# imazen/image-webp

Hardware: AMD Instinct MI355X
Metric: 1920x1080 lossy encodes/s (Q75, method 4) (higher is better)
Workload: dtype int32; 1 GPU; encode_frame_lossy 1920x1080 RGBA Q75 m4; device_batch=1024, distinct_frames=4, mbs_per_frame=8160, parallelism=frames sharded over 1 GPU(s), steps_pipelined=True, pipeline_lanes=2

## Files before the change

image-webp_amd/csrc/zw_enc_kernels.hip:

```cpp
#include "zw_dev.h"

#include "zw_enc_rows.h"

#ifdef ZW_NW
#define ZW_NW1 ZW_NW
#define ZW_NW2 ZW_NW
#endif
#ifndef ZW_NW1
#define ZW_NW1 12
#endif
#ifndef ZW_NW2
#define ZW_NW2 12
#endif
#define NW_MAX (ZW_NW1 > ZW_NW2 ? ZW_NW1 : ZW_NW2)
#ifndef ZW_DYN_PRIO
#define ZW_DYN_PRIO 1
#endif
#ifndef ZW_DYN_PRIO1
#define ZW_DYN_PRIO1 2
#endif
#ifndef ZW_P1_LUMA_MAX
#define ZW_P1_LUMA_MAX 3
#endif
#ifndef ZW_CHAIN_PRIO
#define ZW_CHAIN_PRIO 3
#endif
#ifndef ZW_LUMA_PRIO
#define ZW_LUMA_PRIO 0
#endif
#ifndef ZW_UVQ_CHAIN_ROWS
#define ZW_UVQ_CHAIN_ROWS 1
#endif
#ifndef ZW_UVQ_CHAIN_BATCH
#define ZW_UVQ_CHAIN_BATCH 0
#endif
#ifndef ZW_PAIR_UNROLL
#define ZW_PAIR_UNROLL 1
#endif
#ifndef ZW_FETCH_AHEAD
#define ZW_FETCH_AHEAD (PASS == 2)
#endif
#ifndef ZW_AN4_GPW
#define ZW_AN4_GPW 1
#endif

template <int PASS> struct PassShape {
    static constexpr int NW = PASS == 1 ? ZW_NW1 : ZW_NW2;
    static constexpr int WG = NW * 64;
};

__device__ __forceinline__ int rgb_y(const uint8_t* p)
{
    return (16839 * p[0] + 33059 * p[1] + 6420 * p[2] + (1 << 15) + (16 << 16)) >> 16;
}
__device__ __forceinline__ int rgb_u(const uint8_t* p) { return -9719 * p[0] - 19081 * p[1] + 28800 * p[2] + (128 << 16); }
__device__ __forceinline__ int rgb_v(const uint8_t* p) { return 28800 * p[0] - 24116 * p[1] - 4684 * p[2] + (128 << 16); }

__device__ __forceinline__ void rgb2yuv_sample(const uint8_t* __restrict__ im, int w, int h, int bpp, int mbw, int cx,
                                               int cy, uint8_t* __restrict__ Yf, uint8_t* __restrict__ Uf,
                                               uint8_t* __restrict__ Vf)
{
    const int cw = mbw * 8, lw = mbw * 16;
    const int acw = (w + 1) / 2, ach = (h + 1) / 2;
    const int scx = cx < acw ? cx : acw - 1, scy = cy < ach ? cy : ach - 1;
    int xs[2] = {min(2 * scx, w - 1), min(2 * scx + 1, w - 1)};
    int ys[2] = {min(2 * scy, h - 1), min(2 * scy + 1, h - 1)};
#pragma unroll
    for (int dy = 0; dy < 2; dy++)
#pragma unroll
        for (int dx = 0; dx < 2; dx++) {
            int px = min(2 * cx + dx, w - 1), py = min(2 * cy + dy, h - 1);
            const uint8_t* p = im + ((size_t)py * w + px) * bpp;
            Yf[(size_t)(2 * cy + dy) * lw + 2 * cx + dx] = (uint8_t)(bpp <= 2 ? p[0] : rgb_y(p));
        }
    uint8_t uo = 127, vo = 127;
    if (bpp > 2) {
        int su = 0, sv = 0;
#pragma unroll
        for (int dy = 0; dy < 2; dy++)
#pragma unroll
            for (int dx = 0; dx < 2; dx++) {
                const uint8_t* p = im + ((size_t)ys[dy] * w + xs[dx]) * bpp;
                su += rgb_u(p);
                sv += rgb_v(p);
            }
        uo = (uint8_t)((su + (1 << 17)) >> 18);
        vo = (uint8_t)((sv + (1 << 17)) >> 18);
    }
    Uf[(size_t)cy * cw + cx] = uo;
    Vf[(size_t)cy * cw + cx] = vo;
}

extern "C" __global__ void k_rgb2yuv(const uint8_t* __restrict__ img, int w, int h, int bpp, int mbw, int mbh,
                                     uint8_t* __restrict__ Y, uint8_t* __restrict__ U, uint8_t* __restrict__ V,
                                     size_t img_stride, size_t ysz, size_t csz)
{
    const int cw = mbw * 8, chh = mbh * 8;
    const int f = blockIdx.y;
    const int idx = blockIdx.x * blockDim.x + threadIdx.x;
    if (idx >= cw * chh) return;
    rgb2yuv_sample(img + (size_t)f * img_stride, w, h, bpp, mbw, idx % cw, idx / cw, Y + (size_t)f * ysz,
                   U + (size_t)f * csz, V + (size_t)f * csz);
}

template <int BPP>
__device__ __forceinline__ void rgb_run8(const uint8_t* __restrict__ row, uint32_t px[8])
{
    typedef uint32_t u32x4 __attribute__((ext_vector_type(4)));
    typedef uint32_t u32x2 __attribute__((ext_vector_type(2)));
    if (BPP == 4) {
        const u32x4 a = __builtin_nontemporal_load((const u32x4*)row);
        const u32x4 b = __builtin_nontemporal_load((const u32x4*)(row + 16));
        px[0] = a.x; px[1] = a.y; px[2] = a.z; px[3] = a.w;
        px[4] = b.x; px[5] = b.y; px[6] = b.z; px[7] = b.w;
    } else {
        const u32x2 a = __builtin_nontemporal_load((const u32x2*)row);
        const u32x2 b = __builtin_nontemporal_load((const u32x2*)(row + 8));
        const u32x2 c = __builtin_nontemporal_load((const u32x2*)(row + 16));
        const uint32_t wd[6] = {a.x, a.y, b.x, b.y, c.x, c.y};
#pragma unroll
        for (int q = 0; q < 2; q++) {
            const uint32_t w0 = wd[3 * q], w1 = wd[3 * q + 1], w2 = wd[3 * q + 2];
            px[4 * q] = w0;
            px[4 * q + 1] = __builtin_amdgcn_alignbyte(w1, w0, 3);
            px[4 * q + 2] = __builtin_amdgcn_alignbyte(w2, w1, 2);
            px[4 * q + 3] = w2 >> 8;
        }
    }
}

template <int BPP>
__global__ __launch_bounds__(256) void k_rgb2yuv_rows(const uint8_t* __restrict__ img, int w, int h, int mbw, int mbh,
                                                      uint8_t* __restrict__ Y, uint8_t* __restrict__ U,
                                                      uint8_t* __restrict__ V, size_t img_stride, size_t ysz,
                                                      size_t csz)
{
    const int cw = mbw * 8, chh = mbh * 8, lw = mbw * 16, gpr = mbw * 2;
    const int f = blockIdx.y;
    const int idx = blockIdx.x * blockDim.x + threadIdx.x;
    if (idx >= gpr * chh) return;
    const int g = idx % gpr, cy = idx / gpr;
    const int cx0 = 4 * g, px0 = 8 * g;
    const uint8_t* im = img + (size_t)f * img_stride;
    uint8_t* Yf = Y + (size_t)f * ysz;
    uint8_t* Uf = U + (size_t)f * csz;
    uint8_t* Vf = V + (size_t)f * csz;
    if (px0 + 8 <= w && cy < (h + 1) / 2) {
        const int r0 = 2 * cy, r1 = min(2 * cy + 1, h - 1);
        uint32_t a[8], b[8];
        rgb_run8<BPP>(im + ((size_t)r0 * w + px0) * BPP, a);
        rgb_run8<BPP>(im + ((size_t)r1 * w + px0) * BPP, b);
        const uint32_t ya[2] = {pk_y4(a[0], a[1], a[2], a[3]), pk_y4(a[4], a[5], a[6], a[7])};
        const uint32_t yb[2] = {pk_y4(b[0], b[1], b[2], b[3]), pk_y4(b[4], b[5], b[6], b[7])};
        uint32_t uw = 0, vw = 0;
#pragma unroll
        for (int j = 0; j < 4; j++) {
            const int su = pk_u(a[2 * j]) + pk_u(a[2 * j + 1]) + pk_u(b[2 * j]) + pk_u(b[2 * j + 1]) + (512 << 16);
            const int sv = pk_v(a[2 * j]) + pk_v(a[2 * j + 1]) + pk_v(b[2 * j]) + pk_v(b[2 * j + 1]) + (512 << 16);
            uw |= (uint32_t)((su + (1 << 17)) >> 18) << (8 * j);
            vw |= (uint32_t)((sv + (1 << 17)) >> 18) << (8 * j);
        }
        *(uint2*)(Yf + (size_t)(2 * cy) * lw + px0) = make_uint2(ya[0], ya[1]);
        *(uint2*)(Yf + (size_t)(2 * cy + 1) * lw + px0) = make_uint2(yb[0], yb[1]);
        *(uint32_t*)(Uf + (size_t)cy * cw + cx0) = uw;
        *(uint32_t*)(Vf + (size_t)cy * cw + cx0) = vw;
    } else {
#pragma unroll
        for (int j = 0; j < 4; j++) rgb2yuv_sample(im, w, h, BPP, mbw, cx0 + j, cy, Yf, Uf, Vf);
    }
}

struct AnalysisTile {
    uint32_t y[16][4];
    uint32_t c[2][8][2];
    uint32_t ytop[4], ctop[2][2];
    uint8_t yleft[16], cleft[2][8];
    uint8_t corner[4];
};

DI void an_item(const AnalysisTile* A, bool luma, int mode, int b, bool ht, bool hl, int bins[16], int& z, int& vmax)
{
    const int pl = b >> 2;
    const int bb = luma ? b : (b & 3);
    const int bx = luma ? (bb & 3) : (bb & 1), by = luma ? (bb >> 2) : (bb >> 1);
    uint32_t st = 0, sl = 0;
    if (luma) {
#pragma unroll
        for (int w = 0; w < 4; w++) {
            st = __builtin_amdgcn_sad_u8(A->ytop[w], 0u, st);
            sl = __builtin_amdgcn_sad_u8(((const uint32_t*)A->yleft)[w], 0u, sl);
        }
    } else {
#pragma unroll
        for (int w = 0; w < 2; w++) {
            st = __builtin_amdgcn_sad_u8(A->ctop[pl][w], 0u, st);
            sl = __builtin_amdgcn_sad_u8(((const uint32_t*)A->cleft[pl])[w], 0u, sl);
        }
    }
    const uint32_t s2 = ht && hl ? st + sl : (ht ? 2 * st : 2 * sl);
    const int dcv = (ht || hl) ? (luma ? (int)((s2 + 16) >> 5) : (int)((s2 + 8) >> 4)) : 0x80;
    const int corner = A->corner[luma ? 0 : 1 + pl];
    int d[16];
#pragma unroll
    for (int i = 0; i < 4; i++) {
        const int r = by * 4 + i;
        const uint32_t srow = luma ? A->y[r][bx] : A->c[pl][r][bx];
        const int L = luma ? A->yleft[r] : A->cleft[pl][r];
#pragma unroll
        for (int j = 0; j < 4; j++) {
            const int cidx = bx * 4 + j;
            const uint32_t tw = luma ? A->ytop[cidx >> 2] : A->ctop[pl][cidx >> 2];
            const int T = (int)((tw >> (8 * (cidx & 3))) & 255u);
            const int tm = (ht && hl) ? clamp255(L + T - corner) : (hl ? L : (ht ? T : 129));
            const int p = mode == 0 ? dcv : tm;
            d[i * 4 + j] = (int)((srow >> (8 * j)) & 255u) - p;
        }
    }
    int o[16];
    fdct16_pk(d, o);
    z = 0;
    vmax = 0;
#pragma unroll
    for (int k = 0; k < 16; k++) {
        bins[k] = min(iabs(o[k]) >> 3, 31);
        z += bins[k] == 0;
        vmax = max(vmax, bins[k]);
    }
}
DI int max8(int v)
{
    v = max(v, DPP(v, 0xB1));
    v = max(v, DPP(v, 0x4E));
    return max(v, DPP(v, 0x141));
}
DI int an_red8(int v)
{
    v += DPP(v, 0xB1);
    v += DPP(v, 0x4E);
    return v + DPP(v, 0x141);
}
DI int max16(int v)
{
    v = max8(v);
    return max(v, DPP(v, 0x140));
}
typedef unsigned an_v4u __attribute__((ext_vector_type(4)));
typedef unsigned an_v2u __attribute__((ext_vector_type(2)));
extern "C" __global__ __launch_bounds__(256) void k_analysis4(const uint8_t* __restrict__ Y, const uint8_t* __restrict__ U,
                                                              const uint8_t* __restrict__ V, int mbw, int mbh,
                                                              size_t ysz, size_t csz, uint8_t* __restrict__ alpha,
                                                              uint32_t* __restrict__ histo)
{
    __shared__ AnalysisTile tile[4][4];
    __shared__ uint32_t hist[4][4][4][32];
    __shared__ uint32_t ahist[256];
    const int wv = threadIdx.x >> 6, lane = threadIdx.x & 63, mi = lane >> 4, j = lane & 15;
    const int f = blockIdx.y;
    const int nmb = mbw * mbh;
    ahist[threadIdx.x] = 0;
    __syncthreads();
    const int ys = mbw * 16, cs = mbw * 8;
    const uint8_t* Yf = Y + (size_t)f * ysz;
    const uint8_t* Uf = U + (size_t)f * csz;
    const uint8_t* Vf = V + (size_t)f * csz;
    AnalysisTile* A = &tile[wv][mi];
#pragma unroll 1
    for (int it = 0; it < ZW_AN4_GPW; it++) {
        const int mb = ((blockIdx.x * ZW_AN4_GPW + it) * 4 + wv) * 4 + mi;
        const bool in = mb < nmb;
        const int mbx = in ? mb % mbw : 0, mby = in ? mb / mbw : 0;
        const bool ht = mby > 0, hl = mbx > 0;
        {
            const int pl = j >> 3, cr = j & 7;
            const uint8_t* Cf = pl ? Vf : Uf;
            an_v4u yr = {0u, 0u, 0u, 0u};
            an_v2u cw = {0u, 0u};
            uint32_t yl = 0, cl = 0;
            if (in) {
                const uint8_t* yp = Yf + (size_t)(mby * 16 + j) * ys + mbx * 16;
                const uint8_t* cp = Cf + (size_t)(mby * 8 + cr) * cs + mbx * 8;
                yr = *(const an_v4u*)yp;
                cw = *(const an_v2u*)cp;
                if (hl) {
                    yl = yp[-1];
                    cl = cp[-1];
                }
            }
            wsync();
            *(an_v4u*)A->y[j] = yr;
            *(an_v2u*)A->c[pl][cr] = cw;
            A->yleft[j] = (uint8_t)yl;
            A->cleft[pl][cr] = (uint8_t)cl;
            if (j < 6) {
                uint32_t t0 = 0, t1 = 0, t2 = 0, t3 = 0;
                if (in && ht) {
                    if (j == 0) {
                        const an_v4u t = *(const an_v4u*)(Yf + (size_t)(mby * 16 - 1) * ys + mbx * 16);
                        t0 = t.x; t1 = t.y; t2 = t.z; t3 = t.w;
                    } else if (j < 3) {
                        const an_v2u t = *(const an_v2u*)((j == 1 ? Uf : Vf) + (size_t)(mby * 8 - 1) * cs + mbx * 8);
                        t0 = t.x; t1 = t.y;
                    } else if (hl) {
                        const uint8_t* cp = j == 3 ? Yf + (size_t)(mby * 16 - 1) * ys + mbx * 16 - 1
// ... 2092 lines not shown

struct MbFetch {
    uint32_t y, c;
    int alpha;
};
__device__ __forceinline__ MbFetch fetch_mb(const EncArgs* a, int f, int lane, int mbx, int mby)
{
    const int ys = a->mbw * 16, cs = a->mbw * 8;
    const uint8_t* sy = a->Y + (size_t)f * a->ysz + (size_t)mby * 16 * ys + mbx * 16;
    MbFetch r;
    r.y = *(const uint32_t*)(sy + (size_t)(lane >> 2) * ys + (lane & 3) * 4);
    r.c = 0;
    if (lane < 32) {
        const int pl = lane >> 4, k = lane & 15;
        const uint8_t* sp = (pl ? a->V : a->U) + (size_t)f * a->csz + (size_t)mby * 8 * cs + mbx * 8;
        r.c = *(const uint32_t*)(sp + (size_t)(k >> 1) * cs + (k & 1) * 4);
    }
    r.alpha = a->alpha[(size_t)f * a->mbw * a->mbh + (size_t)mby * a->mbw + mbx];
    return r;
}

__device__ void setup_ctx(Ctx& C, const EncArgs* a, const uint8_t* seg_lut, WaveLds* W, int mbx, int mby,
                          const MbFetch& m)
{
    C.mbx = mbx;
    C.mby = mby;
    const int f = C.f;
    C.ys = a->mbw * 16;
    C.cs = a->mbw * 8;
    C.srcY = a->Y + (size_t)f * a->ysz + (size_t)mby * 16 * C.ys + mbx * 16;
    C.srcU = a->U + (size_t)f * a->csz + (size_t)mby * 8 * C.cs + mbx * 8;
    C.srcV = a->V + (size_t)f * a->csz + (size_t)mby * 8 * C.cs + mbx * 8;
    {
        const int l = C.lane;
        ((uint32_t*)C.M->sy)[l] = m.y;
        if (l < 32) ((uint32_t*)((l >> 4) ? C.M->sv : C.M->su))[l & 15] = m.c;
        C.sY = C.M->sy;
        C.sU = C.M->su;
        C.sV = C.M->sv;
    }
    wsync();
    const int seg = __builtin_amdgcn_readfirstlane((int)seg_lut[m.alpha]);
    C.seg = seg;
    C.S = C.Sl + seg;
}

__device__ void wait_row(const int* progress, int wave_of_prev, int need)
{
    while (__hip_atomic_load(&progress[wave_of_prev], __ATOMIC_ACQUIRE, __HIP_MEMORY_SCOPE_WORKGROUP) < need)
        __builtin_amdgcn_s_sleep(1);
}
DI void set_prio(int p)
{
    if (p >= 3) __builtin_amdgcn_s_setprio(3);
    else if (p == 2) __builtin_amdgcn_s_setprio(2);
    else if (p == 1) __builtin_amdgcn_s_setprio(1);
    else __builtin_amdgcn_s_setprio(0);
}
__device__ void publish(int* progress, int wave, int val)
{
    __builtin_amdgcn_fence(__ATOMIC_RELEASE, "workgroup");
    if ((threadIdx.x & 63) == 0) __hip_atomic_store(&progress[wave], val, __ATOMIC_RELEASE, __HIP_MEMORY_SCOPE_WORKGROUP);
    __builtin_amdgcn_wave_barrier();
}


__device__ __forceinline__ int opaque_lane(int lane)
{
    asm volatile("" : "+v"(lane));
    return lane;
}

struct RowsLayout {
    size_t sync, ty, tu, tv, tc, td, frame;
    __host__ __device__ RowsLayout(int mbw, int mbh)
    {
        auto a16 = [](size_t v) { return (v + 15) & ~(size_t)15; };
        sync = 0;
        ty = a16(4 * (4 + (size_t)mbh));
        tu = ty + a16((size_t)mbw * 16 + 16);
        tv = tu + a16((size_t)mbw * 8);
        tc = tv + a16((size_t)mbw * 8);
        td = tc + a16((size_t)mbw * 12);
        frame = td + a16((size_t)mbw * 4);
    }
};
#define ZW_ROWS_HDR 256
#define ZW_ENC_SPIN_MAX (1 << 22)
DI uint32_t ld_sc1(const void* p) { return __hip_atomic_load((const uint32_t*)p, __ATOMIC_RELAXED, __HIP_MEMORY_SCOPE_AGENT); }
DI void st_sc1(void* p, uint32_t v) { __hip_atomic_store((uint32_t*)p, v, __ATOMIC_RELAXED, __HIP_MEMORY_SCOPE_AGENT); }
DI int row_ticket(int* ticket)
{
    int t = 0;
    if ((threadIdx.x & 63) == 0) t = atomicAdd(ticket, 1);
    return __builtin_amdgcn_readfirstlane(__shfl(t, 0));
}
DI void row_wait(const int* prog, int need, int* err, int& seen)
{
    if (seen >= need) return;
    int it = 0;
    for (;;) {
        seen = __builtin_amdgcn_readfirstlane((int)ld_sc1(prog));
        if (seen >= need) break;
        __builtin_amdgcn_s_sleep(1);
        if (++it > ZW_ENC_SPIN_MAX || ((it & 1023) == 0 && ld_sc1(err))) {
            if ((threadIdx.x & 63) == 0) atomicOr(err, 1);
            seen = 1 << 30;
            break;
        }
    }
    __builtin_amdgcn_fence(__ATOMIC_ACQUIRE, "agent");
}
DI void row_publish(int* prog, int val)
{
    asm volatile("s_waitcnt vmcnt(0)" ::: "memory");
    if ((threadIdx.x & 63) == 0)
        __hip_atomic_store((uint32_t*)prog, (uint32_t)val, __ATOMIC_RELEASE, __HIP_MEMORY_SCOPE_AGENT);
    __builtin_amdgcn_wave_barrier();
}

template <bool ROWS> struct ChainShape {
    static constexpr int NCH = (ROWS ? ZW_UVQ_CHAIN_ROWS : ZW_UVQ_CHAIN_BATCH) ? 2 : 1;
};
#if ZW_PAIR_UNROLL
#define ZW_PAIR_LOOP _Pragma("unroll")
#else
#define ZW_PAIR_LOOP _Pragma("nounroll")
#endif
template <int PASS> struct RowsShape {
    static constexpr int NW = PASS == 1 ? ChainShape<true>::NCH : 1;
};

constexpr size_t a16(size_t v) { return (v + 15) & ~(size_t)15; }

struct EncLds {
    static constexpr size_t sT = a16(sizeof(LdsTables)), sS = a16(4 * sizeof(ZwSegment)), sL = 256;
    static constexpr size_t sW = a16(sizeof(WaveLds)), sM = a16(sizeof(MbLds));
    size_t sy, su, sv, sc, sd;
    static constexpr size_t sProgress = 64, sXch = 256;
    __host__ __device__ EncLds(int mbw, bool rows, int pass)
    {
        const bool all = !rows, chain = rows && pass == 1;
        sy = all ? (((size_t)mbw * 16 + 48 + 15) & ~(size_t)15) : 0;
        su = sv = all || chain ? (((size_t)mbw * 8 + 48 + 15) & ~(size_t)15) : 0;
        sc = all ? (((size_t)mbw * 12 + 15) & ~(size_t)15) : 0;
        sd = all || chain ? (((size_t)mbw * 4 + 15) & ~(size_t)15) : 0;
    }
    __host__ __device__ size_t bytes(int nw, int fp) const
    {
        return sT * fp + sS * fp + sL * fp + sW * nw + (fp == 2 ? sM * nw : 0) + sProgress + sXch +
               (sy + su + sv + sc + sd) * fp;
    }
};
static_assert(NW_MAX * sizeof(int) <= 64, "the progress words");

DI void row_start(MbLds* M, int lane)
{
    if (lane < 20) M->left_y[lane] = 129;
    if (lane < 12) {
        M->left_u[lane] = 129;
        M->left_v[lane] = 129;
        M->left_c[lane] = 0;
    }
    if (lane < 4) M->left_derr[lane] = 0;
}

template <int PASS> DI void luma_issue_prio(const int* progress, int prevw, int mbx, int mby, int mbw)
{
#if ZW_DYN_PRIO > 0
    int slack = mbw;
    if (mby > 0) {
        const int v = __builtin_amdgcn_readfirstlane(
            __hip_atomic_load(&progress[prevw], __ATOMIC_RELAXED, __HIP_MEMORY_SCOPE_WORKGROUP));
        if ((v >> 16) == mby - 1) slack = (v & 0xffff) - mbx - 1;
    }
    constexpr int dp = PASS == 1 ? ZW_DYN_PRIO1 : ZW_DYN_PRIO;
    const int p = slack >= dp * 3 ? 3 : (slack >= dp * 2 ? 2 : (slack >= dp ? 1 : 0));
    set_prio(PASS == 1 ? min(p, ZW_P1_LUMA_MAX) : p);
#endif
}

template <int PASS, bool ROWS, int FP = 1>
__device__ __forceinline__ void encode_body(const EncArgs& a)
{
    constexpr int NW = ROWS ? RowsShape<PASS>::NW : PassShape<PASS>::NW, WG = NW * 64;
    constexpr int NCH = PASS == 1 ? ChainShape<ROWS>::NCH : 0;
    constexpr bool PAIR = FP == 2;
    static_assert(FP == 1 || (FP == 2 && !ROWS), "frame pairs: the batch kernels");
    constexpr int NCW = PASS == 1 ? (PAIR ? 2 : NCH) : 0;
    extern __shared__ __attribute__((aligned(16))) uint8_t smem[];
    const int f = ROWS ? blockIdx.y : blockIdx.x * FP;
    const int nf = PAIR ? min(2, a.nframes - f) : 1;
    const int wv = __builtin_amdgcn_readfirstlane(threadIdx.x >> 6), lane = threadIdx.x & 63;
    const int mbw = a.mbw, mbh = a.mbh;
    const ZwFrameParams* P = a.params + f;
    const EncLds L(mbw, ROWS, PASS);
    size_t off = 0;
    LdsTables* T = (LdsTables*)(smem + off);
    off += L.sT * FP;
    ZwSegment* Sl = (ZwSegment*)(smem + off);
    off += L.sS * FP;
    uint8_t* seg_lut = smem + off;
    off += L.sL * FP;
    WaveLds* Wall = (WaveLds*)(smem + off);
    off += L.sW * NW;
    MbLds* Mall2 = (MbLds*)(smem + off);
    off += PAIR ? L.sM * NW : 0;
    int* progress = (int*)(smem + off);
    off += L.sProgress;
    int* xch = (int*)(smem + off);
    int* xflag = xch + 48;
    off += L.sXch;
    uint8_t* top_y = smem + off;
    off += L.sy * FP;
    uint8_t* top_u = smem + off;
    off += L.su * FP;
    uint8_t* top_v = smem + off;
    off += L.sv * FP;
    uint8_t* top_c = smem + off;
    off += L.sc * FP;
    int8_t* top_derr = (int8_t*)(smem + off);
    WaveLds* W = (WaveLds*)((uint8_t*)Wall + L.sW * wv);
    const bool chain_wg = PASS == 1 && (ROWS ? blockIdx.x == 0 : wv < NCW);
    const RowsLayout RL(mbw, mbh);
    uint8_t* rb = ROWS ? a.rows + ZW_ROWS_HDR + (size_t)f * RL.frame : nullptr;
    int* rerr = ROWS ? (int*)a.rows : nullptr;
    int* rsync = (int*)rb;

#pragma unroll
    for (int fr = 0; fr < FP; fr++) {
        if (fr >= nf) break;
        const int ff = f + fr;
        const ZwFrameParams* Pf = a.params + ff;
        LdsTables* Tf = (LdsTables*)((uint8_t*)T + L.sT * fr);
        ZwSegment* Sf = (ZwSegment*)((uint8_t*)Sl + L.sS * fr);
        uint8_t* lut = seg_lut + L.sL * fr;
        for (int i = threadIdx.x; i < (int)(sizeof(Tf->lc) / 2); i += WG)
            (&Tf->lc[0][0][0][0])[i] = a.lcost ? (&a.lcost[ff].lc[0][0][0][0])[i] : 0;
        for (int i = threadIdx.x; i < 96; i += WG) {
            (&Tf->eob[0][0][0])[i] = a.lcost ? (&a.lcost[ff].eob[0][0][0])[i] : 0;
            (&Tf->init[0][0][0])[i] = a.lcost ? (&a.lcost[ff].init[0][0][0])[i] : 0;
        }
        for (int i = threadIdx.x; i < 4 * 8 * 3 * 11; i += WG) (&Tf->probs[0][0][0][0])[i] = (&Pf->probs[0][0][0][0])[i];
        static_assert(sizeof(ZwSegment) % 4 == 0, "segment copy by dwords");
        for (int i = threadIdx.x; i < (int)(4 * sizeof(ZwSegment) / 4); i += WG)
            ((uint32_t*)Sf)[i] = ((const uint32_t*)Pf->seg)[i];
        for (int i = threadIdx.x; i < 256; i += WG) lut[i] = Pf->seg_enabled ? Pf->seg_map_lut[i] : 0;
        load_static_tables(Tf, threadIdx.x, WG, &Pf->probs[0][0][0][0]);
        if (!ROWS || chain_wg) {
            uint8_t* ty = top_y + L.sy * fr;
            uint8_t* tu = top_u + L.su * fr;
            uint8_t* tv = top_v + L.sv * fr;
            uint8_t* tcx = top_c + L.sc * fr;
            int8_t* td = top_derr + L.sd * fr;
            if (!ROWS) {
                for (int i = threadIdx.x; i < mbw * 16 + 48; i += WG) ty[i] = 127;
                for (int i = threadIdx.x; i < mbw * 12; i += WG) tcx[i] = 0;
            }
            for (int i = threadIdx.x; i < mbw * 8 + 48; i += WG) {
                tu[i] = 127;
                tv[i] = 127;
            }
            for (int i = threadIdx.x; i < mbw * 4; i += WG) td[i] = PASS == 2 ? a.derr[(size_t)ff * mbw * 4 + i] : 0;
        }
    }
    if (threadIdx.x < NW) progress[threadIdx.x] = -1;
    if (threadIdx.x < 2) xflag[threadIdx.x] = 0;
    if (ROWS && lane < 12) W->win_c[lane] = 0;
    __syncthreads();

    Ctx C;
    C.a = &a;
    C.P = P;
    C.T = T;
    C.W = W;
    C.M = &W->mb;
    C.lane = lane;
    C.f = f;
    C.Sl = Sl;
    C.method = __builtin_amdgcn_readfirstlane(P->method);
    C.top_y = top_y;
    C.top_u = top_u;
    C.top_v = top_v;
    C.top_c = top_c;
    C.top_derr = top_derr;
    C.oy = C.oc = C.ocx = C.od = 0;
    const bool trel = PASS == 2 && __builtin_amdgcn_readfirstlane(P->do_trellis);
    const bool keep_i4 = !trel && (PASS == 1 || a.dbg == nullptr);
    const size_t nmb = (size_t)mbw * mbh;
#ifdef ZW_PHASE_PROF
    if (lane < 24) W->ph[lane] = 0;
    wsync();
    auto ph_flush = [&]() {
        if (lane < 24) atomicAdd(&zw_phase_cycles_dev[PASS - 1][lane], W->ph[lane]);
        if (lane < 24) atomicAdd(&zw_wave_cycles_dev[PASS - 1][wv][lane], W->ph[lane]);
    };
#else
    auto ph_flush = []() {};
#endif

    if (chain_wg) {
        __builtin_amdgcn_s_setprio(ZW_CHAIN_PRIO);
        const int cfr = PAIR ? wv : 0;
        if (PAIR && cfr >= nf) {
            ph_flush();
            return;
        }
        const int fc = f + cfr;
        const uint8_t* const lutc = seg_lut + L.sL * cfr;
        int8_t* const tdc = top_derr + L.sd * cfr;
        if (PAIR) {
            C.f = fc;
            C.P = a.params + fc;
            C.T = (const LdsTables*)((const uint8_t*)T + L.sT * cfr);
            C.Sl = (const ZwSegment*)((const uint8_t*)Sl + L.sS * cfr);
            C.top_u = top_u + L.su * cfr;
            C.top_v = top_v + L.sv * cfr;
            C.top_derr = tdc;
            C.method = __builtin_amdgcn_readfirstlane(C.P->method);
        }
        if (lane < 4) C.M->left_derr[lane] = 0;
        if (NCH == 2 && !PAIR) {
            const int pl = wv;
            UvQ U;
            U.pl = pl;
            U.w = W->cu;
            U.sp = C.M->su;
            U.top = pl ? top_v : top_u;
            U.left = C.M->left_u;
            const uint8_t* const P0 = (pl ? a.V : a.U) + (size_t)f * a.csz;
            const int cs = mbw * 8;
            auto fetch_uv = [&](int mbx, int mby) {
                MbFetch r;
                r.y = lane < 16 ? *(const uint32_t*)(P0 + (size_t)(mby * 8 + (lane >> 1)) * cs + mbx * 8 + (lane & 1) * 4)
                                : 0u;
                r.c = 0;
                r.alpha = a.alpha[(size_t)f * nmb + (size_t)mby * mbw + mbx];
                return r;
            };
            C.ys = mbw * 16;
            C.cs = cs;
            MbFetch nx = fetch_uv(0, 0);
            int seq = 0;
            for (int mby = 0; mby < mbh; mby++) {
                if (lane < 12) C.M->left_u[lane] = 129;
                wsync();
                for (int mbx = 0; mbx < mbw; mbx++) {
                    PH_START();
                    const int lane = opaque_lane(threadIdx.x & 63);
                    C.lane = lane;
                    const MbFetch cur = nx;
                    if (mbx + 1 < mbw) nx = fetch_uv(mbx + 1, mby);
                    else if (mby + 1 < mbh) nx = fetch_uv(0, mby + 1);
                    C.mbx = mbx;
                    C.mby = mby;
                    if (lane < 16) ((uint32_t*)C.M->su)[lane] = cur.y;
                    wsync();
                    const int seg = __builtin_amdgcn_readfirstlane((int)seg_lut[cur.alpha]);
                    C.seg = seg;
                    C.S = C.Sl + seg;
                    uvq_border(C, U);
                    const int cm = uvq_pick(C, U, xch, xflag, ++seq);
                    PH_MARK(8);
                    uvq_final(C, U, cm, top_derr + mbx * 4);
                    PH_MARK(9);
                    uvq_store_borders(C, U);
                    ZwMbOut* o = a.out + (size_t)f * nmb + (size_t)mby * mbw + mbx;
                    if (pl == 0 && lane == 0) o->chroma_mode = (uint8_t)cm;
                    write_levels(C, 17 + 4 * pl, 4, false);
                    wsync();
                }
            }
            for (int i = lane; i < mbw * 2; i += 64) {
                const int j = (i >> 1) * 4 + pl * 2 + (i & 1);
                a.derr[(size_t)f * mbw * 4 + j] = top_derr[j];
            }
            ph_flush();
            return;
        }
        MbFetch nx = fetch_mb(&a, fc, lane, 0, 0);
        for (int mby = 0; mby < mbh; mby++) {
            if (lane < 12) {
                C.M->left_u[lane] = 129;
                C.M->left_v[lane] = 129;
            }
            wsync();
            for (int mbx = 0; mbx < mbw; mbx++) {
                PH_START();
                const int lane = opaque_lane(threadIdx.x & 63);
                C.lane = lane;
                const MbFetch cur = nx;
                if (mbx + 1 < mbw) nx = fetch_mb(&a, fc, lane, mbx + 1, mby);
                else if (mby + 1 < mbh) nx = fetch_mb(&a, fc, lane, 0, mby + 1);
                setup_ctx(C, &a, lutc, W, mbx, mby, cur);
                C.oc = mbx * 8;
                C.ocx = mbx * 12;
                build_chroma_border(C);
                const int cm = pick_uv<PASS>(C);
                PH_MARK(8);
                int uvnz[8];
                final_chroma(C, cm, tdc + mbx * 4, uvnz);
                PH_MARK(9);
                store_chroma_borders(C);
                ZwMbOut* o = a.out + (size_t)fc * nmb + (size_t)mby * mbw + mbx;
                if (lane == 0) o->chroma_mode = (uint8_t)cm;
                write_levels(C, 17, 8, false);
                wsync();
            }
        }
        for (int i = lane; i < mbw * 4; i += 64) a.derr[(size_t)fc * mbw * 4 + i] = tdc[i];
        ph_flush();
        return;
    }

    if (PASS == 1) __builtin_amdgcn_s_setprio(ZW_LUMA_PRIO);
    using RS = RowSchedule<PASS, ROWS, NW, NCH>;
    constexpr bool skip_mode = RS::skip_mode;
    constexpr int nrw = RS::nrw;
    const int rw = ROWS ? 0 : RS::first_row(wv, mbh);
    if (ROWS) {
        C.top_y = W->win_y;
        C.top_u = W->win_u;
        C.top_v = W->win_v;
        C.top_c = W->win_c;
        C.top_derr = W->win_d;
    }
    auto mb_store = [&](Ctx& C, int lm, int cm, bool i4reuse, uint32_t i4nz, bool trel) __attribute__((always_inline)) {
        const int lane = C.lane;
        PH_START();
        int ynz[16];
        const int lnz = final_luma(C, lm, trel, ynz, i4reuse ? (int)i4nz : -1);
        PH_MARK(4);
        int uvnz[8] = {0, 0, 0, 0, 0, 0, 0, 0};
        int cnz = 0;
        if (PASS == 2) cnz = final_chroma(C, cm, C.top_derr + C.od, uvnz);
        PH_MARK(5);
        ZwMbOut* o = a.out + (size_t)C.f * nmb + (size_t)C.mby * mbw + C.mbx;
        if (PASS == 2) {
            const int skip = !(lnz | cnz);
            if (lane == 0) {
                uint8_t* tc = C.top_c + C.ocx;
                uint8_t* lc = C.M->left_c;
                if (skip) {
                    for (int k = 1; k < 9; k++) tc[k] = lc[k] = 0;
                    if (lm != 4) tc[0] = lc[0] = 0;
                } else {
                    if (lm != 4) {
                        int y2nz = 0;
                        for (int n = 0; n < 16; n++) y2nz |= C.M->lev[16][n] != 0;
                        tc[0] = lc[0] = (uint8_t)y2nz;
                    }
                    for (int x = 0; x < 4; x++) tc[1 + x] = (uint8_t)ynz[12 + x];
                    for (int y = 0; y < 4; y++) lc[1 + y] = (uint8_t)ynz[y * 4 + 3];
                    tc[5] = (uint8_t)uvnz[2];
                    tc[6] = (uint8_t)uvnz[3];
                    lc[5] = (uint8_t)uvnz[1];
                    lc[6] = (uint8_t)uvnz[3];
                    tc[7] = (uint8_t)uvnz[6];
                    tc[8] = (uint8_t)uvnz[7];
                    lc[7] = (uint8_t)uvnz[5];
                    lc[8] = (uint8_t)uvnz[7];
                }
                o->skip = (uint8_t)skip;
                o->chroma_mode = (uint8_t)cm;
            }
            store_chroma_borders(C);
            write_levels(C, 0, 25, skip);
            if (a.sizes) {
                int e = 0;
                if (lane < 25 && !skip) {
                    const uint32_t* lw = (const uint32_t*)C.M->lev[lane];
#pragma unroll
                    for (int q = 0; q < 8; q++) {
                        const uint32_t v = lw[q];
                        e = (v >> 16) ? 2 * q + 2 : ((v & 0xffffu) ? 2 * q + 1 : e);
                    }
                }
                const int r16 = red16(e);
                const int es = __builtin_amdgcn_readlane(r16, 0) + __builtin_amdgcn_readlane(r16, 16);
                if (lane == 0)
                    a.sizes[(size_t)C.f * nmb + (size_t)C.mby * mbw + C.mbx] = (uint32_t)(1 + (lm == 4 ? 8 : 0) + 25 + 2 * es);
            }
        } else {
            write_levels(C, 0, 17, false);
            if (lane == 0) o->skip = 0;
        }
        if (lane == 0) {
            o->luma_mode = (uint8_t)lm;
            o->segment = (uint8_t)C.seg;
        }
        if (lane < 16) o->bpred[lane] = lm == 4 ? C.M->modes[lane] : 0;
        store_luma_borders(C);
    };
    if constexpr (PAIR) {
        MbLds* const Mp[2] = {&W->mb, Mall2 + wv};
        const int meth0 = C.method;
        const int K = C.method <= 3 ? 3 : (C.method == 4 ? 4 : 10);
        const int meth1 = nf == 2 ? __builtin_amdgcn_readfirstlane(a.params[f + 1].method) : C.method;
        const bool trel1 = PASS == 2 && nf == 2 && __builtin_amdgcn_readfirstlane(a.params[f + 1].do_trellis);
        const bool keep1 = !trel1 && (PASS == 1 || a.dbg == nullptr);
        using RP = RowSchedule<PASS, ROWS, NW, NCW, true>;
        const bool same_k = nf == 1 || (meth1 == C.method && trel1 == trel);
        for (int it = 0;; it++) {
            const int mby = RP::first_row(wv, mbh) + it * RP::nrw;
            if (mby >= mbh) break;
#pragma unroll
            for (int fr = 0; fr < 2; fr++) row_start(Mp[fr], lane);
            wsync();
            const int prevw = mby > 0 ? RP::wave_of_row(mby - 1) : 0;
            auto wait_above = [&](int need) {
                if (mby > 0) wait_row(progress, prevw, (mby - 1) * 65536 + need);
            };
            for (int mbx = 0; mbx < mbw; mbx++) {
                PH_START();
                const int lane = opaque_lane(threadIdx.x & 63);
                C.lane = lane;
                auto enter = [&](int fr) {
                    C.lane = opaque_lane(threadIdx.x & 63);
                    C.f = f + fr;
                    C.P = a.params + C.f;
                    C.T = (const LdsTables*)((const uint8_t*)T + L.sT * fr);
                    C.Sl = (const ZwSegment*)((const uint8_t*)Sl + L.sS * fr);
                    C.top_y = top_y + L.sy * fr;
                    C.top_u = top_u + L.su * fr;
                    C.top_v = top_v + L.sv * fr;
                    C.top_c = top_c + L.sc * fr;
                    C.top_derr = top_derr + L.sd * fr;
                    C.M = fr ? Mp[1] : Mp[0];
                    C.method = fr ? meth1 : meth0;
                    C.mbx = mbx;
                    C.mby = mby;
                    C.oy = mbx * 16;
                    C.oc = mbx * 8;
                    C.ocx = mbx * 12;
                    C.od = mbx * 4;
                    C.sY = C.M->sy;
                    C.sU = C.M->su;
                    C.sV = C.M->sv;
                };
                auto pst = [&](int fr, int k) { return (uint32_t)__builtin_amdgcn_readfirstlane((int)W->pst[fr][k]); };
                wait_above(min(mbx + 1, mbw));
                luma_issue_prio<PASS>(progress, prevw, mbx, mby, mbw);
                PH_MARK(0);
ZW_PAIR_LOOP
                for (int fr = 0; fr < 2; fr++) {
                    if (fr >= nf) {
                        if (lane == 0) W->pst[fr][0] = 0;
                        continue;
                    }
                    enter(fr);
                    const MbFetch fm = fetch_mb(&a, C.f, lane, mbx, mby);
                    setup_ctx(C, &a, seg_lut + L.sL * fr, W, mbx, mby, fm);
                    build_luma_border(C, 0);
                    int l_;
                    unsigned long long s_;
                    pick_i16<PASS>(C, l_, s_);
                    const bool n_ = C.method > 1 && (C.method >= 5 || s_ > 211ull * C.S->l_mode || l_ != 0);
                    if (lane == 0) {
                        W->pst[fr][0] = (uint32_t)l_ | ((uint32_t)n_ << 4) | ((uint32_t)C.seg << 8);
                        W->pst[fr][1] = (uint32_t)s_;
                        W->pst[fr][2] = (uint32_t)(s_ >> 32);
                        W->pst[fr][3] = 0;
                    }
                    wsync();
                }
                wsync();
                PH_MARK(1);
                const uint32_t s0 = pst(0, 0), s1 = pst(1, 0);
                const bool n0 = (s0 >> 4) & 1u, n1 = (s1 >> 4) & 1u;
                if (n0 || n1) wait_above(min(mbx + 2, mbw));
ZW_PAIR_LOOP
                for (int fr = 0; fr < 2; fr++) {
                    if (!((pst(fr, 0) >> 4) & 1u)) continue;
                    enter(fr);
                    build_luma_border(C, 1);
                }
                PH_MARK(21);
                if (K <= 4 && same_k && (n0 || n1)) {
                    Ctx CA = C, CB = C;
                    CA.lane = CB.lane = opaque_lane(threadIdx.x & 63);
                    CA.T = T;
                    CB.T = (const LdsTables*)((const uint8_t*)T + L.sT);
                    CA.M = Mp[0];
                    CB.M = Mp[1];
                    CA.S = Sl + (s0 >> 8);
                    CB.S = (const ZwSegment*)((const uint8_t*)Sl + L.sS) + (s1 >> 8);
                    CA.sY = Mp[0]->sy;
                    CB.sY = Mp[1]->sy;
                    const unsigned long long i0 = pst(0, 1) | ((unsigned long long)pst(0, 2) << 32);
                    const unsigned long long i1 = pst(1, 1) | ((unsigned long long)pst(1, 2) << 32);
                    uint32_t z0 = 0, z1 = 0;
                    const uint32_t r = pick_i4_pair<PASS>(CA, CB, i0, i1, n0, n1, keep_i4, z0, z1);
                    if (lane == 0) {
                        W->pst[0][3] = (r & 1u) ? (z0 | 0x10000u) : 0u;
                        W->pst[1][3] = (r & 2u) ? (z1 | 0x10000u) : 0u;
                    }
                } else if (n0 || n1) {
ZW_PAIR_LOOP
                    for (int fr = 0; fr < 2; fr++) {
                        const uint32_t sm = pst(fr, 0);
                        if (!((sm >> 4) & 1u)) continue;
                        enter(fr);
                        C.seg = (int)(sm >> 8);
                        C.S = C.Sl + C.seg;
                        uint32_t z = 0;
                        const bool w4 = pick_i4<PASS>(C, pst(fr, 1) | ((unsigned long long)pst(fr, 2) << 32),
                                                      fr ? keep1 : keep_i4, z);
                        if (lane == 0) W->pst[fr][3] = w4 ? (z | 0x10000u) : 0u;
                    }
                }
                wsync();
                PH_MARK(2);
ZW_PAIR_LOOP
                for (int fr = 0; fr < 2; fr++) {
                    if (fr >= nf) continue;
                    enter(fr);
                    const uint32_t sm = pst(fr, 0), r4 = pst(fr, 3);
                    C.seg = (int)(sm >> 8);
                    C.S = C.Sl + C.seg;
                    int cm = 0;
                    if (PASS == 2) {
                        build_chroma_border(C);
                        cm = pick_uv<PASS>(C);
                    }
                    PH_MARK(3);
                    const bool w4 = (r4 >> 16) & 1u;
                    mb_store(C, w4 ? 4 : (int)(sm & 15u), cm, w4 && (fr ? keep1 : keep_i4), r4 & 0xffffu,
                             fr ? trel1 : trel);
                    PH_RESET();
                }
                publish(progress, wv, mby * 65536 + mbx + 1);
                PH_MARK(6);
            }
        }
        ph_flush();
        return;
    }
    uint8_t* const gty = ROWS ? rb + RL.ty : nullptr;
    uint8_t* const gtu = ROWS ? rb + RL.tu : nullptr;
    uint8_t* const gtv = ROWS ? rb + RL.tv : nullptr;
    uint8_t* const gtc = ROWS ? rb + RL.tc : nullptr;
    uint8_t* const gtd = ROWS ? rb + RL.td : nullptr;
    for (int it = 0, yk = rw;; it++) {
        const int mby = ROWS ? row_ticket(&rsync[0]) : (skip_mode ? yk : rw + it * nrw);
        if (skip_mode) yk = RS::next_row(wv, yk, mbh);
        if (mby >= mbh) break;
        row_start(C.M, lane);
        wsync();
        const int prevw = (!ROWS && mby > 0) ? RS::wave_of_row(mby - 1) : 0;
        int seen = -1;
        int* const prog_above = ROWS ? rsync + 4 + (mby > 0 ? mby - 1 : 0) : nullptr;
        auto wait_above = [&](int need) {
            if (mby == 0) return;
            if (ROWS) row_wait(prog_above, need, rerr, seen);
            else wait_row(progress, prevw, (mby - 1) * 65536 + need);
        };
        MbFetch nx;
        if (ZW_FETCH_AHEAD) nx = fetch_mb(&a, f, lane, 0, mby);
        for (int mbx = 0; mbx < mbw; mbx++) {
            PH_START();
            const int lane = opaque_lane(threadIdx.x & 63);
            C.lane = lane;
            MbFetch cur;
            if (ZW_FETCH_AHEAD) {
                cur = nx;
                if (mbx + 1 < mbw) nx = fetch_mb(&a, f, lane, mbx + 1, mby);
            } else {
                cur = fetch_mb(&a, f, lane, mbx, mby);
            }
            wait_above(min(mbx + 1, mbw));
            if (ROWS) {
                if (mby > 0) {
                    uint32_t v = 0;
                    if (lane < 4) v = ld_sc1(gty + mbx * 16 + 4 * lane);
                    else if (PASS == 2 && lane < 6) v = ld_sc1(gtu + mbx * 8 + 4 * (lane - 4));
                    else if (PASS == 2 && lane < 8) v = ld_sc1(gtv + mbx * 8 + 4 * (lane - 6));
                    else if (PASS == 2 && lane < 11) v = ld_sc1(gtc + mbx * 12 + 4 * (lane - 8));
                    else if (PASS == 2 && lane < 12) v = ld_sc1(gtd + mbx * 4);
                    if (lane < 4) ((uint32_t*)W->win_y)[lane] = v;
                    else if (PASS == 2 && lane < 6) ((uint32_t*)W->win_u)[lane - 4] = v;
                    else if (PASS == 2 && lane < 8) ((uint32_t*)W->win_v)[lane - 6] = v;
                    else if (PASS == 2 && lane < 11) ((uint32_t*)W->win_c)[lane - 8] = v;
                    else if (PASS == 2 && lane < 12) ((uint32_t*)W->win_d)[0] = v;
                } else if (PASS == 2) {
                    if (lane < 3) ((uint32_t*)W->win_c)[lane] = 0;
                    else if (lane == 3)
                        ((uint32_t*)W->win_d)[0] = *(const uint32_t*)(a.derr + (size_t)f * mbw * 4 + mbx * 4);
                }
                wsync();
            } else {
                C.oy = mbx * 16;
                C.oc = mbx * 8;
                C.ocx = mbx * 12;
                C.od = mbx * 4;
            }
            if (!ROWS) luma_issue_prio<PASS>(progress, prevw, mbx, mby, mbw);
            PH_MARK(0);
            setup_ctx(C, &a, seg_lut, W, mbx, mby, cur);
            build_luma_border(C, 0);
            int lm;
            unsigned long long i16s;
            pick_i16<PASS>(C, lm, i16s);
            wsync();
            PH_MARK(1);
            int cm = 0;
            uint32_t i4nz = 0;
            bool i4reuse = false;
            if (PASS == 2) {
                build_chroma_border(C);
                cm = pick_uv<PASS>(C);
            }
            PH_MARK(3);
            if (C.method > 1) {
                const unsigned long long thr = 211ull * C.S->l_mode;
                if (C.method >= 5 || i16s > thr || lm != 0) {
                    wait_above(min(mbx + 2, mbw));
                    if (ROWS && mby > 0 && mbx + 1 < mbw) {
                        uint32_t v = 0;
                        if (lane < 4) v = ld_sc1(gty + (mbx + 1) * 16 + 4 * lane);
                        if (lane < 4) ((uint32_t*)W->win_y)[4 + lane] = v;
                        wsync();
                    }
                    build_luma_border(C, 1);
                    PH_MARK(21);
                    if (pick_i4<PASS>(C, i16s, keep_i4, i4nz)) {
                        lm = 4;
                        i4reuse = keep_i4;
                    }
                }
            }
            PH_MARK(2);
            mb_store(C, lm, cm, i4reuse, i4nz, trel);
            PH_RESET();
            if (ROWS) {
                if (mby + 1 < mbh) {
                    if (lane < 4) st_sc1(gty + mbx * 16 + 4 * lane, ((const uint32_t*)W->win_y)[lane]);
                    else if (PASS == 2 && lane < 6) st_sc1(gtu + mbx * 8 + 4 * (lane - 4), ((const uint32_t*)W->win_u)[lane - 4]);
                    else if (PASS == 2 && lane < 8) st_sc1(gtv + mbx * 8 + 4 * (lane - 6), ((const uint32_t*)W->win_v)[lane - 6]);
                    else if (PASS == 2 && lane < 11) st_sc1(gtc + mbx * 12 + 4 * (lane - 8), ((const uint32_t*)W->win_c)[lane - 8]);
                    else if (PASS == 2 && lane < 12) st_sc1(gtd + mbx * 4, ((const uint32_t*)W->win_d)[0]);
                    row_publish(rsync + 4 + mby, mbx + 1);
                }
            } else {
                publish(progress, wv, mby * 65536 + mbx + 1);
            }
            PH_MARK(6);
        }
    }
    ph_flush();
}

extern "C" __global__ __launch_bounds__(PassShape<1>::WG) void k_encode_pass1(EncArgs a) { encode_body<1, false>(a); }
extern "C" __global__ __launch_bounds__(PassShape<1>::WG) void k_encode_pass1_fp(EncArgs a) { encode_body<1, false, 2>(a); }
extern "C" __global__ __launch_bounds__(PassShape<2>::WG) void k_encode_pass2(EncArgs a) { encode_body<2, false>(a); }
extern "C" __global__ __launch_bounds__(PassShape<2>::WG) void k_encode_pass2_fp(EncArgs a) { encode_body<2, false, 2>(a); }
extern "C" __global__ __launch_bounds__(64 * RowsShape<1>::NW) void k_encode_rows_pass1(EncArgs a) { encode_body<1, true>(a); }
extern "C" __global__ __launch_bounds__(64) void k_encode_rows_pass2(EncArgs a) { encode_body<2, true>(a); }

struct QuantBlocksArgs {
    ZwMatrix m;
    uint16_t sharpen[16];
    uint32_t lambda;
    int32_t ctype, first, trel, n;
};

extern "C" __global__ __launch_bounds__(256) void k_quant_blocks(const int* __restrict__ coeffs,
                                                                const uint8_t* __restrict__ ctx0s,
                                                                const ZwLevelCosts* __restrict__ lcost,
                                                                const uint8_t* __restrict__ probs, QuantBlocksArgs a,
                                                                int* __restrict__ levels, int* __restrict__ dq)
{
    __shared__ LdsTables T;
    for (int i = threadIdx.x; i < (int)(sizeof(T.lc) / 2); i += 256) (&T.lc[0][0][0][0])[i] = (&lcost->lc[0][0][0][0])[i];
    for (int i = threadIdx.x; i < 96; i += 256) {
        (&T.eob[0][0][0])[i] = (&lcost->eob[0][0][0])[i];
        (&T.init[0][0][0])[i] = (&lcost->init[0][0][0])[i];
    }
    for (int i = threadIdx.x; i < 4 * 8 * 3 * 11; i += 256) (&T.probs[0][0][0][0])[i] = probs[i];
    load_static_tables(&T, threadIdx.x, 256, probs);
    __syncthreads();
    const int b = blockIdx.x * 256 + threadIdx.x;
    if (b >= a.n) return;
    int c[16], lv[16];
#pragma unroll
    for (int k = 0; k < 16; k++) c[k] = coeffs[(size_t)b * 16 + k];
    const int ctx0 = ctx0s[b];
    if (a.trel) {
        if (a.first) trellis<1>(c, lv, a.m, a.sharpen, a.lambda, &T, a.ctype, ctx0);
        else trellis<0>(c, lv, a.m, a.sharpen, a.lambda, &T, a.ctype, ctx0);
        if (a.first) lv[0] = 0;
    } else {
#pragma unroll
        for (int n = 0; n < 16; n++) {
            const int j = kZZ(n);
            lv[n] = n < a.first ? 0 : quantz(c[j], a.m.iq[j > 0], a.m.bias[j > 0]);
        }
#pragma unroll
        for (int n = 0; n < 16; n++) {
            const int j = kZZ(n);
            c[j] = n < a.first ? 0 : m24(lv[n], (int)a.m.q[j > 0]);
        }
    }
#pragma unroll
    for (int k = 0; k < 16; k++) {
        levels[(size_t)b * 16 + k] = lv[k];
        dq[(size_t)b * 16 + k] = c[k];
    }
}

extern "C" __global__ __launch_bounds__(256) void k_quant_blocks_g(const int* __restrict__ coeffs,
                                                                  const uint8_t* __restrict__ ctx0s,
                                                                  const ZwLevelCosts* __restrict__ lcost,
// ... 169 lines not shown
```

image-webp_amd/csrc/zw_enc_rows.h:

```cpp
#pragma once

#ifndef ZW_HD
#ifdef __HIPCC__
#define ZW_HD __host__ __device__
#else
#define ZW_HD
#endif
#endif

#ifndef ZW_P1_ORDER
#define ZW_P1_ORDER 1
#endif
#ifndef ZW_P1_SLOWSKIP
#define ZW_P1_SLOWSKIP 1
#endif
#ifndef ZW_P1_SLOW_NUM
#define ZW_P1_SLOW_NUM 1
#endif
#ifndef ZW_P1_SLOW_DEN
#define ZW_P1_SLOW_DEN 1
#endif

template <int PASS, bool ROWS, int NW, int NCH, bool PAIR = false> struct RowSchedule {
    static_assert(PASS == 1 || NCH == 0, "chain waves are pass 1's");
    static constexpr bool plain = PASS == 2 || PAIR;
    static constexpr int nrw = NW - NCH;
    static constexpr bool skip_mode = ZW_P1_SLOWSKIP && PASS == 1 && !ROWS && !PAIR && NCH == 1 && NW > 4;
    static constexpr int nslow = (NW - 1) / 4 > 0 ? (NW - 1) / 4 : 1;
    static constexpr int nfast = NW - NCH - (NW - 1) / 4;

    static ZW_HD bool p1_before(int v, int w)
    {
        const bool sv = (v & 3) < NCH, sw = (w & 3) < NCH;
        return (ZW_P1_ORDER && sv != sw) ? sw : v < w;
    }
    static ZW_HD int luma_rank(int w)
    {
        if (plain) return w - NCH;
        int r = 0;
        for (int v = NCH; v < NW; v++) r += (int)p1_before(v, w);
        return r;
    }
    static ZW_HD int luma_wave(int k)
    {
        if (plain) return k + NCH;
        int w = NCH;
        for (int v = NCH; v < NW; v++)
            if (luma_rank(v) == k) w = v;
        return w;
    }
    static ZW_HD int fast_wave(int i) { return i + 1 + i / 3; }
    static ZW_HD int wave_of_row(int y)
    {
        if (!skip_mode) return luma_wave(y % (nrw > 0 ? nrw : 1));
        constexpr int L = ZW_P1_SLOW_DEN * nfast + ZW_P1_SLOW_NUM;
        int r = y % L, before = (y / L) * ZW_P1_SLOW_NUM;
        for (int k = 0; k < ZW_P1_SLOW_DEN; k++) {
            const int sk = ((k + 1) * ZW_P1_SLOW_NUM) / ZW_P1_SLOW_DEN - (k * ZW_P1_SLOW_NUM) / ZW_P1_SLOW_DEN;
            if (r < nfast) return fast_wave(r);
            r -= nfast;
            if (r < sk) return 4 * (1 + (before + r) % nslow);
            r -= sk;
            before += sk;
        }
        return 0;
    }
    static ZW_HD int next_row(int wave, int y, int mbh)
    {
        if (!skip_mode) return y + nrw;
        for (y++; y < mbh; y++)
            if (wave_of_row(y) == wave) break;
        return y;
    }
    static ZW_HD int first_row(int wave, int mbh) { return skip_mode ? next_row(wave, -1, mbh) : luma_rank(wave); }
};
```

Baseline: 4437 encodes/s.

## Add pass-1 pair row schedule where chain waves join luma rows late

In the paired-frame pass 1 kernel, chain waves no longer return after their chroma chain finishes. They fall through and take luma rows. A new PairRowSchedule1 gives fast and slow waves different row shares up to a join row, then deals the remaining rows round-robin across all waves, including the former chain waves. The aim is to cut the idle time of chain-SIMD waves and rebalance work across SIMDs, at the cost of more complex row-to-wave mapping and the risk of dependency stalls at the join point.

```diff
diff --git a/image-webp_amd/csrc/zw_enc_kernels.hip b/image-webp_amd/csrc/zw_enc_kernels.hip
--- a/image-webp_amd/csrc/zw_enc_kernels.hip
+++ b/image-webp_amd/csrc/zw_enc_kernels.hip
@@ -1,4 +1,6 @@
 #include "zw_dev.h"
+
+#include <type_traits>
 
 #include "zw_enc_rows.h"
 
@@ -2697,11 +2699,8 @@
     if (chain_wg) {
         __builtin_amdgcn_s_setprio(ZW_CHAIN_PRIO);
         const int cfr = PAIR ? wv : 0;
-        if (PAIR && cfr >= nf) {
-            ph_flush();
-            return;
-        }
-        const int fc = f + cfr;
+        const bool has_chain = !PAIR || cfr < nf;
+        const int fc = f + (has_chain ? cfr : 0);
         const uint8_t* const lutc = seg_lut + L.sL * cfr;
         int8_t* const tdc = top_derr + L.sd * cfr;
         if (PAIR) {
@@ -2774,7 +2773,7 @@
             return;
         }
         MbFetch nx = fetch_mb(&a, fc, lane, 0, 0);
-        for (int mby = 0; mby < mbh; mby++) {
+        for (int mby = 0; has_chain && mby < mbh; mby++) {
             if (lane < 12) {
                 C.M->left_u[lane] = 129;
                 C.M->left_v[lane] = 129;
@@ -2803,9 +2802,19 @@
                 wsync();
             }
         }
-        for (int i = lane; i < mbw * 4; i += 64) a.derr[(size_t)fc * mbw * 4 + i] = tdc[i];
-        ph_flush();
-        return;
+        for (int i = lane; has_chain && i < mbw * 4; i += 64) a.derr[(size_t)fc * mbw * 4 + i] = tdc[i];
+        if (!PAIR) {
+            ph_flush();
+            return;
+        }
+        C.f = f;
+        C.P = P;
+        C.T = T;
+        C.Sl = Sl;
+        C.top_u = top_u;
+        C.top_v = top_v;
+        C.top_derr = top_derr;
+        C.method = __builtin_amdgcn_readfirstlane(P->method);
     }
 
     if (PASS == 1) __builtin_amdgcn_s_setprio(ZW_LUMA_PRIO);
@@ -2894,15 +2903,14 @@
         const int meth1 = nf == 2 ? __builtin_amdgcn_readfirstlane(a.params[f + 1].method) : C.method;
         const bool trel1 = PASS == 2 && nf == 2 && __builtin_amdgcn_readfirstlane(a.params[f + 1].do_trellis);
         const bool keep1 = !trel1 && (PASS == 1 || a.dbg == nullptr);
-        using RP = RowSchedule<PASS, ROWS, NW, NCW, true>;
+        using RP =
+            typename std::conditional<PASS == 1, PairRowSchedule1<NW, NCW>, RowSchedule<PASS, ROWS, NW, NCW, true>>::type;
         const bool same_k = nf == 1 || (meth1 == C.method && trel1 == trel);
-        for (int it = 0;; it++) {
-            const int mby = RP::first_row(wv, mbh) + it * RP::nrw;
-            if (mby >= mbh) break;
+        for (int mby = RP::first_row(wv, mbh); mby < mbh; mby = RP::next_row(wv, mby, mbh)) {
 #pragma unroll
             for (int fr = 0; fr < 2; fr++) row_start(Mp[fr], lane);
             wsync();
-            const int prevw = mby > 0 ? RP::wave_of_row(mby - 1) : 0;
+            const int prevw = mby > 0 ? RP::wave_of_row(mby - 1, mbh) : 0;
             auto wait_above = [&](int need) {
                 if (mby > 0) wait_row(progress, prevw, (mby - 1) * 65536 + need);
             };
diff --git a/image-webp_amd/csrc/zw_enc_rows.h b/image-webp_amd/csrc/zw_enc_rows.h
--- a/image-webp_amd/csrc/zw_enc_rows.h
+++ b/image-webp_amd/csrc/zw_enc_rows.h
@@ -65,6 +65,7 @@
         }
         return 0;
     }
+    static ZW_HD int wave_of_row(int y, int ) { return wave_of_row(y); }
     static ZW_HD int next_row(int wave, int y, int mbh)
     {
         if (!skip_mode) return y + nrw;
@@ -74,3 +75,103 @@
     }
     static ZW_HD int first_row(int wave, int mbh) { return skip_mode ? next_row(wave, -1, mbh) : luma_rank(wave); }
 };
+
+#ifndef ZW_P1P_SLOW_NUM
+#define ZW_P1P_SLOW_NUM 4
+#endif
+#ifndef ZW_P1P_SLOW_DEN
+#define ZW_P1P_SLOW_DEN 1
+#endif
+#ifndef ZW_P1P_JOIN_NUM
+#define ZW_P1P_JOIN_NUM 5
+#endif
+#ifndef ZW_P1P_JOIN_DEN
+#define ZW_P1P_JOIN_DEN 8
+#endif
+#ifndef ZW_P1P_JOIN_MIN
+#define ZW_P1P_JOIN_MIN 24
+#endif
+
+template <int NW, int NCH> struct PairRowSchedule1 {
+    static_assert(NW % 4 == 0 && NW > 4 && NW <= 16 && NCH >= 1 && NCH < 4, "chain waves on some of the four SIMDs");
+    static_assert(ZW_P1P_SLOW_NUM >= 0 && ZW_P1P_SLOW_DEN >= 1, "the slow-row share");
+    static_assert(ZW_P1P_JOIN_NUM >= 0 && ZW_P1P_JOIN_NUM <= ZW_P1P_JOIN_DEN && ZW_P1P_JOIN_DEN >= 1, "the join fraction");
+    static constexpr int nslow = (NW / 4 - 1) * NCH;
+    static constexpr int nfast = NW - NCH - nslow;
+    static constexpr int L = ZW_P1P_SLOW_DEN * nfast + ZW_P1P_SLOW_NUM;
+    static constexpr int span = L * nslow;
+
+    static ZW_HD int join_row(int mbh)
+    {
+        return mbh < ZW_P1P_JOIN_MIN ? mbh : (mbh * ZW_P1P_JOIN_NUM + ZW_P1P_JOIN_DEN - 1) / ZW_P1P_JOIN_DEN;
+    }
+    static ZW_HD int fast_wave(int i) { return (i / (4 - NCH)) * 4 + NCH + i % (4 - NCH); }
+    static ZW_HD int slow_wave(int i) { return 4 * (1 + i / NCH) + i % NCH; }
+    static ZW_HD int round_wave(int y)
+    {
+        int r = y % L, before = (y / L) * ZW_P1P_SLOW_NUM;
+        for (int k = 0; k < ZW_P1P_SLOW_DEN; k++) {
+            const int sk = ((k + 1) * ZW_P1P_SLOW_NUM) / ZW_P1P_SLOW_DEN - (k * ZW_P1P_SLOW_NUM) / ZW_P1P_SLOW_DEN;
+            if (r < nfast) return fast_wave(r);
+            r -= nfast;
+            if (r < sk) return slow_wave((before + r) % nslow);
+            r -= sk;
+            before += sk;
+        }
+        return NCH;
+    }
+    static ZW_HD unsigned long long join_scan(int J, unsigned& seen, int& n)
+    {
+        unsigned long long ord = 0;
+        seen = 0;
+        n = 0;
+        for (int y = J - 1; y >= 0 && y >= J - span; y--) {
+            const int w = round_wave(y);
+            if (!((seen >> w) & 1u)) {
+                seen |= 1u << w;
+                ord |= (unsigned long long)w << (4 * n++);
+            }
+        }
+        return ord;
+    }
+    static ZW_HD int join_rank(int wave, int J)
+    {
+        unsigned seen;
+        int n;
+        const unsigned long long ord = join_scan(J, seen, n);
+        if ((seen >> wave) & 1u) {
+            int i = 0;
+            while ((int)((ord >> (4 * i)) & 15u) != wave) i++;
+            return NW - 1 - i;
+        }
+        int r = 0;
+        for (int v = 0; v < wave; v++) r += (int)!((seen >> v) & 1u);
+        return r;
+    }
+    static ZW_HD int join_wave(int k, int J)
+    {
+        unsigned seen;
+        int n;
+        const unsigned long long ord = join_scan(J, seen, n);
+        if (k >= NW - n) return (int)((ord >> (4 * (NW - 1 - k))) & 15u);
+        int w = 0;
+        for (;; w++)
+            if (!((seen >> w) & 1u) && k-- == 0) break;
+        return w;
+    }
+    static ZW_HD int wave_of_row(int y, int mbh)
+    {
+        const int J = join_row(mbh);
+        return y < J ? round_wave(y) : join_wave((y - J) % NW, J);
+    }
+    static ZW_HD int next_row(int wave, int y, int mbh)
+    {
+        const int J = join_row(mbh);
+        for (y++; y < J; y++)
+            if (round_wave(y) == wave) return y;
+        if (y >= mbh) return y;
+        const int k = join_rank(wave, J);
+        return y + (k - (y - J) % NW + NW) % NW;
+    }
+    static ZW_HD int first_row(int wave, int mbh) { return next_row(wave, -1, mbh); }
+};
```

After: 4485 encodes/s, median of 6. +1.1%, better.
